# alebal123bal/BayesOpt_smart

Hardware: AMD Instinct MI355X
Metric: candidate-points/sec (GP predict + HVI) at N_train=512, N_cand=1M (higher is better)
Workload: dtype f64; 1 GPU; C3: 2D/2-obj toy_function, N_train=512, N_cand=1,048,576 per GPU ('ij' integer grid), HVI (Sigma-UCB), q=3; n_train=512, n_cand_per_gpu=1048576, n_cand_total=1048576, n_objectives=2, dim=2, topq=3, parallelism=candidate-shard x1, step_launch=hip_graph, candidate_offset=0

## Files before the change

### bayesopt_smart_amd/csrc/bo_gridconv.hip

```cpp

#include "bo_predict_impl.h"

namespace {

using namespace bo;

constexpr int kListWaves = 4;
constexpr int kListChunk = 512;
#ifndef BO_ACC_RB
#define BO_ACC_RB 8
#endif
constexpr int kAccRB = BO_ACC_RB;
constexpr int kAccRows = 64 * kAccRB;
constexpr int kAccUnroll = 4;
constexpr int kClassLists = kConvClasses * kConvShards;
static_assert(kClassLists % 64 == 0 && kClassLists <= 2 * 64 * kConvAccWaves &&
              (kConvShards & (kConvShards - 1)) == 0 && kConvShards <= 16 && kConvShards <= kConvCountStride,
              "conv_acc_kernel's scan and lookup of the class lists");
constexpr int kConvPF = 3;
constexpr size_t kConvLdsBytes = 160 * 1024;
constexpr double kPairDrop = 0x1p-100;
constexpr double kTabFlush = 0x1p-128;

struct ListLds {
  int order, rc, nm;
  size_t bytes;
  __host__ __device__ ListLds(int n, int C)
      : order(C + 1), rc(order + n), nm(rc + 2 * n), bytes((size_t)(nm + kListWaves * kListChunk) * sizeof(int)) {}
};
struct AccLds {
  int ints, part;
  size_t bytes;
  __host__ __device__ explicit AccLds(int R)
      : ints(4 * R), part(kClassLists + 1),
        bytes((size_t)ints * sizeof(double) + (size_t)(part + kConvAccWaves + 1) / 2 * 2 * sizeof(int)) {}
};
struct ContractLds {
  int HB, tabH, hband, cn;
  size_t bytes;
  __host__ __device__ ContractLds(int C, int Cpad, int LT, int NP)
      : HB(Cpad + LT / 2), tabH(2 * HB), hband(tabH + Cpad + C - 1), cn(hband + 1),
        bytes((size_t)cn * sizeof(double) + (size_t)NP * sizeof(int)) {}
};

__device__ __forceinline__ void conv_list_done(const ConvArgs& a, int tau, int kept, int lane, int dyn) {
  if (kept == 0) {
    for (int o = 0; o < a.n_obj; ++o) {
      double* row = a.T + ((size_t)o * a.LT + tau) * a.ldr;
      for (int i = lane; i < a.ldr; i += 64) row[i] = 0.0;
    }
  }
  if (lane == 0) {
    a.pkept[tau] = kept;
    if (dyn && kept > 0) {
      const int e = 31 - __clz(kept);
      const int cls = 2 * e + (e > 0 ? (kept >> (e - 1)) & 1 : 0);
      const int sh = tau & (kConvShards - 1);
      const int slot = atomicAdd(a.ccount + cls * kConvCountStride + sh, 1);
      a.clist[(size_t)(cls * kConvShards + sh) * (a.LT / kConvShards) + slot] = tau;
    }
  }
}

__global__ __launch_bounds__(64 * kListWaves) void conv_list_kernel(const ConvArgs a, int tau_blocks, int dyn) {
  if (__builtin_amdgcn_readfirstlane(*a.flag) != 0) return;
  const int tid = threadIdx.x;
  if ((int)blockIdx.x >= tau_blocks) {
    const long long total = (long long)a.NP * a.ldr;
    const long long stride = (long long)(gridDim.x - tau_blocks) * (64 * kListWaves);
    for (int o = 0; o < a.n_obj; ++o) {
      const double nhl = a.nhl[o], pv = a.pv[o];
      double* tm = a.Tm + (size_t)o * a.NP * a.ldr;
      for (long long t = (long long)(blockIdx.x - tau_blocks) * (64 * kListWaves) + tid; t < total; t += stride) {
        const int s = (int)(t / a.ldr), i = (int)(t - (long long)s * a.ldr);
        double v = 0.0;
        if (s < a.n && i < a.nrows) {
          const int n = a.order[s];
          const double d = (double)(a.row_lo + i - a.rc[2 * n]);
          v = pv * a.alpha[(size_t)o * a.n_pad + n] * exp(nhl * (d * d));
        }
        tm[t] = v;
      }
    }
    return;
  }
  extern __shared__ __attribute__((aligned(16))) int si[];
  const ListLds L(a.n, a.C);
  int* cstart = si;
  int* order = si + L.order;
  int* rc = si + L.rc;
  for (int t = tid; t <= a.C; t += 64 * kListWaves) cstart[t] = a.cstart[t];
  for (int t = tid; t < a.n; t += 64 * kListWaves) order[t] = a.order[t];
  for (int t = tid; t < 2 * a.n; t += 64 * kListWaves) rc[t] = a.rc[t];
  __syncthreads();
  const int lane = tid & 63, wave = tid >> 6;
// ... 185 lines not shown
    int incl = sum;
#pragma unroll
    for (int d = 1; d < 64; d <<= 1) {
      const int v = __shfl_up(incl, d, 64);
      if (lane >= d) incl += v;
    }
    if (lane == 63) part[tid >> 6] = incl;
    __syncthreads();
    int run = incl - sum;
    for (int w = 0; w < (tid >> 6); ++w) run += part[w];
#pragma unroll
    for (int u = 0; u < 2; ++u) {
      const int j = 2 * tid + u;
      if (j < kClassLists) cst[j] = run;
      run += c[u];
      if (j == kClassLists - 1) cst[kClassLists] = run;
    }
  }
  __syncthreads();
  const int n_items = (dyn ? cst[kClassLists] : a.LT) * nrb;
  const double* wo = pair_w + (size_t)o * a.n_pairs;
  const int g = blockIdx.x % ngrp;
  int* tk = ticket + (o * kConvTicketGroups + g) * kConvTicketStride;
  for (int k = (blockIdx.x / ngrp) * kConvAccWaves + (tid >> 6);;) {
    const int t = k * ngrp + g;
    if (t >= n_items) break;
    int nx = 0;
    if (dyn && lane == 0) nx = atomicAdd(tk, 1);
    const int oi = t / nrb, rb = t - oi * nrb;
    int tau = oi;
    if (dyn) {
      constexpr int per = kClassLists / 64;
      const unsigned long long b1 = __ballot(cst[per * lane + per] > oi);
      const int l1 = __builtin_ctzll(b1);
      const unsigned long long b2 = __ballot(cst[per * l1 + (lane < per ? lane : per - 1) + 1] > oi);
      const int j = per * l1 + __builtin_ctzll(b2);
      const int cls = kConvClasses - 1 - j / kConvShards;
      const int* list = clist + (size_t)(cls * kConvShards + j % kConvShards) * (a.LT / kConvShards);
      tau = __builtin_amdgcn_readfirstlane(list[oi - cst[j]]);
    }
    const int p0 = __builtin_amdgcn_readfirstlane(pstart[tau]);
    const int cnt = __builtin_amdgcn_readfirstlane(pkept[tau]);
    if (!dyn && cnt == 0) break;
    const int ib = rb * kAccRows;
    double* Trow = T + ((size_t)o * a.LT + tau) * a.ldr;
    if (ib + kAccRows <= a.nrows) conv_acc_item<true>(tabE, wo + p0, pair_sl + p0, cnt, ib, lane, a.nrows, a.ldr, Trow);
    else conv_acc_item<false>(tabE, wo + p0, pair_sl + p0, cnt, ib, lane, a.nrows, a.ldr, Trow);
    if (!dyn) break;
    k = __builtin_amdgcn_readfirstlane(nx);
  }
}

__device__ __forceinline__ void conv_load_a(const double* __restrict__ X, int ldr, int kb, int g, double (&v)[4]) {
  const double* p = X + (size_t)(16 * kb + 4 * g) * ldr;
#pragma unroll
  for (int s = 0; s < 4; ++s) v[s] = p[(size_t)s * ldr];
}

template <class BGen>
__device__ __forceinline__ void conv_gemm(const double* __restrict__ X, int ldr, int nkb, int g, d4 (&acc)[4],
                                          BGen&& bgen) {
  double ring[kConvPF][4];
#pragma unroll
  for (int p = 0; p < kConvPF; ++p) conv_load_a(X, ldr, p < nkb ? p : nkb - 1, g, ring[p]);
  for (int kb0 = 0; kb0 < nkb; kb0 += kConvPF) {
#pragma unroll
    for (int p = 0; p < kConvPF; ++p) {
      const int kb = kb0 + p;
      if (kb < nkb) {
        double av[4];
#pragma unroll
        for (int s = 0; s < 4; ++s) av[s] = ring[p][s];
        const int nx = kb + kConvPF;
        conv_load_a(X, ldr, nx < nkb ? nx : nkb - 1, g, ring[p]);
        double bv[4][4];
        bgen(kb, bv);
#pragma unroll
        for (int s = 0; s < 4; ++s)
#pragma unroll
          for (int nb = 0; nb < 4; ++nb) acc[nb] = mfma64(av[s], bv[s][nb], acc[nb]);
      }
    }
  }
}

__global__ __launch_bounds__(256, 2) void conv_contract_kernel(const ConvArgs a) {
  if (__builtin_amdgcn_readfirstlane(*a.flag) != 0) return;
  extern __shared__ __attribute__((aligned(16))) double sd[];
  const ContractLds L(a.C, a.Cpad, a.LT, a.NP);
  double* tabB = sd;
  double* tabH = sd + L.tabH;
  int* hband = (int*)(sd + L.hband);
  int* cn = (int*)(sd + L.cn);
  const int tid = threadIdx.x, lane = tid & 63, wave = tid >> 6;
  const int g = lane >> 4, jl = lane & 15;
  const int cb_n = a.Cpad / 64;
  const long long n_wt = (long long)(a.ldr / 16) * cb_n;
  const long long gi_lo = a.cand_offset, gi_hi = a.cand_offset + a.n_cand;
  for (int t = tid; t < a.NP; t += 256) cn[t] = t < a.n ? a.rc[2 * a.order[t] + 1] : 0;

  double lv = -__builtin_inf();
  long long li = -1;
  double tab_nhl = __builtin_nan("");
  for (long long base = (long long)blockIdx.x * 4; base < n_wt; base += (long long)gridDim.x * 4) {
    const long long wt = base + wave;
    const bool active = wt < n_wt;
    const long long wtc = active ? wt : n_wt - 1;
    const int i0 = (int)(wtc / cb_n) * 16, j0 = (int)(wtc % cb_n) * 64;
    double acq[4][4];
    for (int o = 0; o < a.n_obj; ++o) {
      const double nhl = a.nhl[o];
      if (!(nhl == tab_nhl)) {
        __syncthreads();
        int mq = 0;
        for (int t = tid; t < 2 * L.HB; t += 256) {
          const int par = t >= L.HB ? 1 : 0, h = t - par * L.HB;
          const int mi = 2 * h + par - (a.LT - 1);
          const double m = (double)mi;
          const double v = exp(0.5 * nhl * (m * m));
          const bool flush = v < kTabFlush;
          tabB[t] = flush ? 0.0 : v;
          if (!flush) mq = max(mq, abs(mi));
        }
        int mm = 0;
        for (int t = tid; t < a.Cpad + a.C - 1; t += 256) {
          const int mi = t - (a.C - 1);
          const double m = (double)mi;
          const double v = exp(nhl * (m * m));
          const bool flush = v < kTabFlush;
          tabH[t] = flush ? 0.0 : v;
          if (!flush) mm = max(mm, abs(mi));
        }
        if (tid < 2) hband[tid] = 0;
        __syncthreads();
#pragma unroll
        for (int d = 32; d > 0; d >>= 1) {
          mq = max(mq, __shfl_xor(mq, d, 64));
          mm = max(mm, __shfl_xor(mm, d, 64));
        }
        if (lane == 0) {
          atomicMax(hband, mq);
          atomicMax(hband + 1, mm);
        }
        __syncthreads();
        tab_nhl = nhl;
      }
      int kq_lo = 0, kq_hi = a.LT / 16;
      if (!a.full) {
        const int hq = hband[0];
        const int t_lo = 2 * j0 - hq > 0 ? 2 * j0 - hq : 0;
        const int t_hi = 2 * (j0 + 63) + hq < a.LT - 1 ? 2 * (j0 + 63) + hq : a.LT - 1;
        kq_lo = __builtin_amdgcn_readfirstlane(t_lo >> 4);
        kq_hi = __builtin_amdgcn_readfirstlane((t_hi >> 4) + 1);
      }
      d4 aq[4], am[4];
#pragma unroll
      for (int nb = 0; nb < 4; ++nb) {
        aq[nb] = (d4){0.0, 0.0, 0.0, 0.0};
        am[nb] = (d4){0.0, 0.0, 0.0, 0.0};
      }
      const double* Tq = a.T + ((size_t)o * a.LT + 16 * kq_lo) * a.ldr + i0 + jl;
      int km_lo = 0, km_hi = a.NP / 16;
      if (!a.full) {
        const int hm = hband[1];
        const int c_lo = j0 - hm > 0 ? j0 - hm : 0, c_hi = j0 + 64 + hm < a.C ? j0 + 64 + hm : a.C;
        km_lo = __builtin_amdgcn_readfirstlane(a.cstart[c_lo] >> 4);
        km_hi = __builtin_amdgcn_readfirstlane((a.cstart[c_hi] + 15) >> 4);
      }
      const double* Tm = a.Tm + ((size_t)o * a.NP + 16 * km_lo) * a.ldr + i0 + jl;
      const double* pe0 = tabB + (a.LT / 2 - 1 - 8 * kq_lo - 2 * g) + j0 + jl;
      conv_gemm(Tq, a.ldr, kq_hi - kq_lo, g, aq, [&](int kb, double (&bv)[4][4]) {
        const double* pe = pe0 - 8 * kb;
        const double* po = pe + L.HB;
#pragma unroll
        for (int nb = 0; nb < 4; ++nb) {
          bv[0][nb] = po[16 * nb];
          bv[1][nb] = pe[16 * nb];
          bv[2][nb] = po[16 * nb - 1];
          bv[3][nb] = pe[16 * nb - 1];
        }
      });
      const int* cn0 = cn + 16 * km_lo + 4 * g;
      if (km_hi > km_lo) conv_gemm(Tm, a.ldr, km_hi - km_lo, g, am, [&](int kb, double (&bv)[4][4]) {
        const int* c4 = cn0 + 16 * kb;
        const double* ph = tabH + j0 + jl + (a.C - 1);
#pragma unroll
        for (int s = 0; s < 4; ++s) {
          const double* p = ph - c4[s];
#pragma unroll
          for (int nb = 0; nb < 4; ++nb) bv[s][nb] = p[16 * nb];
        }
      });
      mfma_fence<false>(aq[0], aq[1]);
      mfma_fence<false>(aq[2], aq[3]);
      mfma_fence<false>(am[0], am[1]);
      mfma_fence<false>(am[2], am[3]);
      const double pv = a.pv[o], pm = a.pm[o];
#pragma unroll
      for (int nb = 0; nb < 4; ++nb) {
#pragma unroll
        for (int r = 0; r < 4; ++r) {
          const double mu = pm + am[nb][r];
          const double var = fmax(pv - aq[nb][r], a.min_var);
          const double smu = (mu - pm) * a.inv_rsq_pv[o];
          const double svar = var * a.inv_pv[o];
          const double u = smu + a.beta[o] * sqrt(fabs(svar));
          acq[nb][r] = (o == 0) ? u : acq[nb][r] + u;
          const int row = a.row_lo + i0 + g + 4 * r, c = j0 + 16 * nb + jl;
          const long long gi = (long long)row * a.C + c;
          if (active && i0 + g + 4 * r < a.nrows && c < a.C && gi >= gi_lo && gi < gi_hi) {
            const long long off = (long long)o * a.ld_out + (gi - gi_lo);
            if (a.mu) bo_out_store(a.mu + off, mu);
            if (a.var) bo_out_store(a.var + off, var);
            if (a.std_mu) bo_out_store(a.std_mu + off, smu);
            if (a.std_var) bo_out_store(a.std_var + off, svar);
            if (a.ucb) bo_out_store(a.ucb + off, u);
          }
        }
      }
    }
    long long gis[4][4];
#pragma unroll
    for (int nb = 0; nb < 4; ++nb) {
#pragma unroll
      for (int r = 0; r < 4; ++r) {
        const int row = a.row_lo + i0 + g + 4 * r, c = j0 + 16 * nb + jl;
        const long long gi = (long long)row * a.C + c;
        const bool ok = active && i0 + g + 4 * r < a.nrows && c < a.C && gi >= gi_lo && gi < gi_hi;
        gis[nb][r] = ok ? gi : -1;
        if (ok && a.acq) bo_out_store(a.acq + (gi - gi_lo), acq[nb][r]);
      }
    }
    if (a.topq > 0) {
      const int q = a.topq;
      const unsigned long long kq = bo_readlane_u(bo_order_key(lv, li), q - 1);
      const long long iq = bo_readlane_i(li, q - 1);
      bool beats = false;
#pragma unroll
      for (int nb = 0; nb < 4; ++nb)
#pragma unroll
        for (int r = 0; r < 4; ++r)
          beats = beats || bo_key_before(bo_order_key(acq[nb][r], gis[nb][r]), gis[nb][r], kq, iq);
      if (__ballot(beats) != 0ull) {
        unsigned int taken = 0;
        double nv = -__builtin_inf();
        long long ni = -1;
        int filled = 0;
        while (filled < q) {
          unsigned long long bk = 0ull;
          long long bi = -1;
          int bs = -1;
#pragma unroll
          for (int nb = 0; nb < 4; ++nb) {
#pragma unroll
            for (int r = 0; r < 4; ++r) {
              const int s = 4 * nb + r;
              const unsigned long long k = ((taken >> s) & 1u) ? 0ull : bo_order_key(acq[nb][r], gis[nb][r]);
              if (bo_key_before(k, gis[nb][r], bk, bi)) { bk = k; bi = gis[nb][r]; bs = s; }
            }
          }
          {
            const unsigned long long k = (lane < q && !((taken >> 16) & 1u)) ? bo_order_key(lv, li) : 0ull;
            if (bo_key_before(k, li, bk, bi)) { bk = k; bi = li; bs = 16; }
          }
          unsigned long long wk = bk;
          long long wi = bi;
#pragma unroll
          for (int m = 32; m > 0; m >>= 1) {
            const unsigned long long ok = __shfl_xor(wk, m, 64);
            const long long oi = __shfl_xor(wi, m, 64);
            if (bo_key_before(ok, oi, wk, wi)) { wk = ok; wi = oi; }
          }
          if (wk == 0ull) break;
          const bool win = bk == wk && bi == wi;
          bool excluded = false;
          if (win) {
            taken |= 1u << bs;
            if (bs != 16) {
              const long long row = wi / a.C, c = wi - row * a.C;
              double co[BO_MAX_DIM] = {(double)(a.lo0 + row), (double)(a.lo1 + c), 0.0, 0.0, 0.0, 0.0, 0.0, 0.0};
              excluded = bo_hash_contains(a.hkeys, a.hidx, a.hmask, a.excl_pts, 2, co, 2);
            }
          }
          if (__ballot(excluded) != 0ull) continue;
          if (lane == filled) { nv = bo_key_value(wk); ni = wi; }
          ++filled;
        }
        lv = nv;
        li = ni;
      }
    }
  }
  if (a.topq > 0) {
    if (lane < a.topq) {
      TopEntry* dst = a.partial + ((size_t)blockIdx.x * 4 + wave) * a.topq;
      dst[lane].v = lv;
      dst[lane].i = li;
    }
    if (blockIdx.x == 0) {
      const long long e0 = (long long)gridDim.x * 4 * a.topq, e1 = (long long)a.n_lists * a.topq;
      for (long long e = e0 + tid; e < e1; e += 256) {
        a.partial[e].v = -__builtin_inf();
        a.partial[e].i = -1;
      }
    }
  }
}

}

namespace bo {

bool conv_lds_admits(int n, int R, int C, int Cpad, int LT, int NP) {
  const size_t bound = ((size_t)4 * R + 2048) * sizeof(double) + ((size_t)(C + 1) + 3 * (size_t)n + 2048) * sizeof(int);
  assert(ConvSetupLds(n, C, 256).bytes <= bound && ListLds(n, C).bytes <= bound && AccLds(R).bytes <= bound);
  return bound <= kConvLdsBytes && ContractLds(C, Cpad, LT, NP).bytes <= kConvLdsBytes;
}

template <class K>
static hipError_t conv_lds_attr(K k, size_t lds) {
  if (lds <= 64 * 1024) return hipSuccess;
  return hipFuncSetAttribute((const void*)k, hipFuncAttributeMaxDynamicSharedMemorySize, (int)lds);
}

ConvSched conv_acc_schedule(int R, int LT, int ldr, int n_obj, int cus) {
  ConvSched sc;
  sc.nrb = (ldr + kAccRows - 1) / kAccRows;
  const long long items = (long long)LT * sc.nrb;
  const size_t tab = (size_t)4 * R * sizeof(double);
  const int per_cu = (int)(kConvLdsBytes / tab < 4 ? kConvLdsBytes / tab : 4);
  long long wgs = (long long)(cus > 0 ? cus : 256) * per_cu / n_obj;
  if (wgs > (items + kConvAccWaves - 1) / kConvAccWaves) wgs = (items + kConvAccWaves - 1) / kConvAccWaves;
  if (wgs < 1) wgs = 1;
  sc.wgs = (int)wgs;
  sc.ngrp = (int)(wgs < kConvTicketGroups ? wgs : kConvTicketGroups);
  sc.dyn = (items <= wgs * kConvAccWaves && wgs % sc.ngrp == 0) ? 0 : 1;
  return sc;
}

hipError_t launch_gridconv(const ConvArgs& ca, int grid, const ConvSched& sc, hipStream_t st) {
  const size_t l1 = ListLds(ca.n, ca.C).bytes, la = AccLds(ca.R).bytes;
  const size_t l2 = ContractLds(ca.C, ca.Cpad, ca.LT, ca.NP).bytes;
  if (l1 > kConvLdsBytes || la > kConvLdsBytes) return hipErrorInvalidValue;
  hipError_t e;
  if ((e = conv_lds_attr(conv_list_kernel, l1)) != hipSuccess) return e;
  if ((e = conv_lds_attr(conv_acc_kernel, la)) != hipSuccess) return e;
  if ((e = conv_lds_attr(conv_contract_kernel, l2)) != hipSuccess) return e;
  const int tau_blocks = (ca.LT + kListWaves - 1) / kListWaves;
  const long long tm_elems = (long long)ca.NP * ca.ldr;
  const int tm_blocks = (int)((tm_elems + 1023) / 1024 < 512 ? (tm_elems + 1023) / 1024 : 512);
  hipLaunchKernelGGL(conv_list_kernel, dim3(tau_blocks + tm_blocks), dim3(64 * kListWaves), l1, st, ca, tau_blocks,
                     sc.dyn);
  if ((e = hipGetLastError()) != hipSuccess) return e;
  hipLaunchKernelGGL(conv_acc_kernel, dim3((unsigned)sc.wgs, ca.n_obj), dim3(64 * kConvAccWaves), la, st, ca,
                     (const double*)ca.pair_w, (const int*)ca.pair_sl, (const int*)ca.pstart, (const int*)ca.pkept,
                     (const int*)ca.ccount, (const int*)ca.clist, ca.ticket, ca.T, sc.nrb, sc.ngrp, sc.dyn);
  if ((e = hipGetLastError()) != hipSuccess) return e;
  hipLaunchKernelGGL(conv_contract_kernel, dim3(grid), dim3(256), l2, st, ca);
  return hipGetLastError();
}

}
```

### bayesopt_smart_amd/csrc/bo_predict.hip

```cpp

#include "bo_predict_impl.h"

#include <vector>

namespace {

__device__ __forceinline__ double kstar_at(const FusedArgs& a, int o, int f, long long j, bool valid) {
  return (valid && f < a.n_train) ? a.kstar[((long long)o * a.ks_rows + f) * a.n_cand + j] : 0.0;
}

template <int NS, bool SELECT>
__device__ __forceinline__ void contract_epair(__amdgpu_buffer_rsrc_t wr, int voff, int base,
                                               int& pos, int ep, const double (&B)[NS],
                                               d2 (&wa)[kPF], d2 (&wb)[kPF], d4& acc0, d4& acc1,
                                               double (&sel0)[4], double (&sel1)[4]) {
  constexpr int NCH = NS / 8;
#pragma unroll
  for (int c = 0; c < NCH; ++c) {
#pragma unroll
    for (int pp = 0; pp < 4; ++pp) {
      const int p = 4 * c + pp;
      const d2 ca = wa[pp];
      const d2 cb = wb[pp];
      const int so = base + ((pos + kPF) << 11);
// ... 353 lines not shown
  if (b < p.alpha_blocks) {
    const long long row_id = (long long)b * 4 + wave;
    if (row_id >= (long long)p.n_obj * p.n_pad) return;
    const int o = (int)(row_id / p.n_pad), f = (int)(row_id % p.n_pad);
    double s = 0.0;
    if (f < p.n) {
      const double* wr = p.kinv + (long long)o * p.ld_k * p.ld_k + (long long)f * p.ld_k;
      const double pm = p.pm[o];
      for (int e = lane; e < p.n; e += 64) s = __builtin_fma(wr[e], p.y[(long long)e * p.ld_y + o] - pm, s);
    }
#pragma unroll
    for (int m = 32; m > 0; m >>= 1) s += __shfl_xor(s, m, 64);
    if (lane == 0) p.alpha[row_id] = s;
    return;
  }
  b -= p.alpha_blocks;
  const long long t0 = (long long)b * 256 + tid, stride = (long long)p.pack_blocks * 256;
  if (p.pack_mode == 0) pack_cm_range(t0, stride, (d2*)p.wpack, p.kinv, p.ld_k, p.upper, p.n, p.n_pad, p.n_obj);
  else if (p.pack_mode == 1) pack_range(t0, stride, (d2*)p.wpack, p.kinv, p.ld_k, p.n, p.n_pad, p.ns, p.n_obj);
  else pack32_range(t0, stride, (f4*)p.wpack, p.kinv, p.ld_k, p.n, p.n_pad, p.n_obj);
}

__global__ void selftest_mfma32_kernel(const float* a, const float* b, float* d) {
  const int l = threadIdx.x;
  const float av = a[(l & 15) * 4 + (l >> 4)];
  const float bv = b[(l >> 4) * 16 + (l & 15)];
  f4 acc = {0.0f, 0.0f, 0.0f, 0.0f};
  acc = mfma32(av, bv, acc);
#pragma unroll
  for (int r = 0; r < 4; ++r) d[(4 * (l >> 4) + r) * 16 + (l & 15)] = acc[r];
}

inline int pad_rows(long long n) { return (int)((n + 31) / 32 * 32); }
inline int pad_dim(int d) { return d <= 2 ? 2 : (d <= 4 ? 4 : (d <= 6 ? 6 : 8)); }
inline size_t align256(size_t x) { return (x + 255) & ~(size_t)255; }
constexpr size_t kLdsBytes = 160 * 1024;
constexpr size_t kLdsDoubles = kLdsBytes / sizeof(double);

int num_cus() {
  static int cus = 0;
  if (cus == 0) {
    int dev = 0;
    if (hipGetDevice(&dev) != hipSuccess) return 256;
    hipDeviceProp_t p;
    if (hipGetDeviceProperties(&p, dev) != hipSuccess) return 256;
    cus = p.multiProcessorCount;
  }
  return cus;
}

constexpr double kConvMargin = 1.15;
constexpr int kConvMaxN = 4096;

void plan_gridconv(const bo_predict_desc* d, Plan* pl, bool kmem) {
  if (kmem || !pl->cm || d->cand_kind != BO_CAND_GRID || d->dim != 2 || d->n_cand <= 0) return;
  if (d->mode & (BO_PREDICT_DENSE | BO_PREDICT_NO_SEPARABLE | BO_PREDICT_FP32 | BO_PREDICT_NO_GRID_CONV)) return;
  const char* env = getenv("BO_GRID_CONV");
  if (env && env[0] == '0' && env[1] == 0) return;
  const long long R = d->grid_shape[0], C = d->grid_shape[1], n = d->n_train;
  if (R < 1 || C < 1 || R > (1 << 15) || C > (1 << 15) || n > kConvMaxN) return;
  if (d->cand_offset < 0 || d->cand_offset + d->n_cand > R * C) return;
  bo::ConvPlan cp = {};
  cp.row_lo = (int)(d->cand_offset / C);
  cp.nrows = (int)((d->cand_offset + d->n_cand - 1) / C) - cp.row_lo + 1;
  cp.ldr = (cp.nrows + 15) / 16 * 16;
  cp.Cpad = (int)((C + 63) / 64 * 64);
  cp.LT = (int)((2 * C - 1 + 15) / 16 * 16);
  cp.NP = (int)((n + 15) / 16 * 16);
  if (!bo::conv_lds_admits((int)n, (int)R, (int)C, cp.Cpad, cp.LT, cp.NP)) return;
  const long long wave_tiles = (long long)(cp.ldr / 16) * (cp.Cpad / 64);
  if (!(d->mode & (BO_PREDICT_GRID_CONV | BO_PREDICT_GRID_CONV_FULL))) {
    const double nch = pl->n_pad / 32;
    const double F = (double)d->n_obj * 1024.0 * nch * (nch + 1);
    const double old_rounds = (double)(((d->n_cand + 63) / 64 + 255) / 256);
    const double old_us = 25.0 + old_rounds * 64.0 * (F / 273.0e3 + 0.038);
    const double pairs_per_tau = 0.5 * (double)n * (double)(n + 1) / (double)(2 * C - 1);
    const double pair_us = 2.2 * pairs_per_tau * (double)((cp.ldr + 1023) / 1024) *
                           (double)((d->n_obj * (2 * C - 1) + 4095) / 4096);
    const double tile_rounds = (double)((wave_tiles + 1023) / 1024);
    const double contract_us = tile_rounds * 2048.0 * (double)(cp.LT + cp.NP) * (double)d->n_obj / 48.8e3;
    const double conv_us = 60.0 + pair_us + contract_us;
    if (!(kConvMargin * conv_us < old_us)) return;
  }
  cp.planned = true;
  const long long wgs = (wave_tiles + 3) / 4;
  cp.grid = (int)(wgs < pl->grid ? wgs : pl->grid);
  cp.ws = bo::conv_layout(n, d->n_obj, C, cp.LT, cp.NP, cp.ldr, align256(pl->total));
  pl->total = cp.ws.end;
  pl->conv = cp;
}

int make_plan(const bo_predict_desc* d, Plan* pl, bool query_device, bool kmem = false) {
  if (!d || d->n_obj < 1 || d->n_obj > BO_MAX_OBJ || d->dim < 1 || d->dim > BO_MAX_DIM)
    return BO_ERR_ARG;
  if (d->n_train < 1 || d->n_cand < 0 || d->topq < 0 || d->topq > BO_MAX_TOPQ) return BO_ERR_ARG;
  if (d->cand_kind < 0 || d->cand_kind > BO_CAND_SOBOL) return BO_ERR_ARG;
  if (d->mode & ~(BO_PREDICT_DENSE | BO_PREDICT_NO_SEPARABLE | BO_PREDICT_FP32 | BO_PREDICT_F32_FLOOR |
                  BO_PREDICT_NO_GRID_CONV | BO_PREDICT_GRID_CONV | BO_PREDICT_GRID_CONV_FULL))
    return BO_ERR_ARG;
  if (d->excl_points && d->n_excl < 0) return BO_ERR_ARG;
  const long long n = d->n_train;
  if (n > (1 << 14)) return BO_ERR_UNSUPPORTED;
  memset(pl, 0, sizeof(*pl));
  pl->dim_pad = pad_dim(d->dim);
  pl->n_excl = (int)(d->excl_points ? d->n_excl : n);
  pl->n_panels = 1;
  if ((d->mode & BO_PREDICT_FP32) && !kmem) {
    const int n_pad = (int)((n + 63) / 64 * 64);
    const size_t lds = ((size_t)n_pad * pl->dim_pad + (size_t)d->n_obj * n_pad) * sizeof(float);
    if (lds <= kLdsBytes) {
      pl->fp32 = true;
      pl->n_pad = n_pad;
      pl->ns = 16;
      pl->lds = lds;
    }
  }
  if (!pl->fp32 && !kmem) {
    const int n_pad = pad_rows(n);
    const size_t base = (size_t)n_pad * pl->dim_pad + (size_t)d->n_obj * n_pad;
    pl->cm = true;
    pl->n_pad = n_pad;
    pl->ns = n_pad / 4;
    const size_t plain = base + bo::kExpTab;
    size_t lds = plain;
    if (d->cand_kind == BO_CAND_GRID && !(d->mode & BO_PREDICT_NO_SEPARABLE)) {
      const long long S = d->grid_shape[d->dim - 1];
      const size_t tbl = (size_t)d->n_obj * (2 * S - 1);
      const size_t rw_c = (size_t)n_pad * (d->n_obj + 1) + (size_t)(S + 63) / 64;
      const size_t lds_c = base + tbl + (size_t)kWaves * rw_c;
      const size_t lds_1 = base + tbl + (size_t)kWaves * n_pad * 2;
      if (S % 16 == 0 && S <= 32768 && d->cand_offset % 16 == 0 && lds_1 <= kLdsDoubles) {
        pl->sep = true;
        pl->rw_cache = lds_c <= kLdsDoubles;
        pl->rw_stride = (int)(pl->rw_cache ? rw_c : (size_t)n_pad * 2);
        pl->off_tbl = (int)base;
        pl->off_rw = (int)(base + tbl);
        lds = pl->rw_cache ? lds_c : lds_1;
        if (lds < plain) lds = plain;
      }
    }
    pl->off_exp = (int)base;
    if (lds > kLdsDoubles) {
      pl->sep = false;
      pl->grows = true;
      pl->off_exp = 0;
      lds = bo::kExpTab;
    }
    pl->lds = lds * sizeof(double);
#ifndef BO_ABL_NOSMALL
    pl->small = !pl->grows && n_pad <= 4 * 32 && pl->lds <= kLdsBytes / 2 - 1024;
#endif
  }
  if (kmem) {
    int n_pad = pad_rows(n);
    int ns;
    bool multi = false;
    if (n_pad <= 32) ns = 8;
    else if (n_pad <= 64) ns = 16;
    else if (n_pad <= 128) ns = 32;
    else if (n_pad <= 256) ns = 64;
    else { ns = bo::kPanelSteps; multi = true; }
    n_pad = multi ? (int)((n + 511) / 512 * 512) : ns * 4;
    pl->n_pad = n_pad;
    pl->ns = ns;
    pl->multi = multi;
    pl->n_panels = multi ? n_pad / 512 : 1;
    pl->lds = (size_t)d->n_obj * n_pad * sizeof(double);
    if (pl->lds > 160 * 1024) return BO_ERR_UNSUPPORTED;
  }
  const int n_pad = pl->n_pad;
  const size_t w_bytes = (size_t)d->n_obj * n_pad * n_pad * sizeof(double);
  if (w_bytes >= (1ull << 31)) return BO_ERR_UNSUPPORTED;
  pl->waves = kWaves;
  const long long n_tiles = (d->n_cand + kTile - 1) / kTile;
  pl->n_tiles = n_tiles;
  const int cus = query_device ? num_cus() : 256;
#ifdef BO_SMALL_ONE_SLOT
  const int slots = cus;
#else
  const int slots = pl->small ? 2 * cus : cus;
#endif
  pl->grid = (int)(n_tiles < slots ? (n_tiles > 0 ? n_tiles : 1) : slots);
  pl->off_alpha = align256(w_bytes);
  pl->off_xpad = pl->off_alpha + align256((size_t)d->n_obj * n_pad * sizeof(double));
  pl->off_xc = pl->off_xpad + align256((size_t)n_pad * pl->dim_pad * sizeof(double));
  pl->off_excl = pl->off_xc + align256((size_t)n_pad * pl->dim_pad * sizeof(double));
  pl->off_hash = pl->off_excl + align256((size_t)(pl->n_excl + 1) * pl->dim_pad * sizeof(double));
  pl->hash_slots = bo_hash_slots(pl->n_excl);
  pl->off_partial = pl->off_hash + align256((size_t)pl->hash_slots * 12);
  pl->off_status = pl->off_partial +
                   align256((size_t)1024 * kWaves * (d->topq > 0 ? d->topq : 1) * sizeof(TopEntry));
  pl->total = pl->off_status + 256 + 256;
  plan_gridconv(d, pl, kmem);
  return BO_OK;
}

template <int NS, bool MULTI>
hipError_t launch_kmem_k(const FusedArgs& fa, int grid, size_t lds, hipStream_t st) {
  auto k = kmem_predict_kernel<NS, MULTI>;
  if (lds > 64 * 1024) {
    hipError_t e = hipFuncSetAttribute((const void*)k, hipFuncAttributeMaxDynamicSharedMemorySize,
                                       (int)lds);
    if (e != hipSuccess) return e;
  }
  hipLaunchKernelGGL(k, dim3(grid), dim3(256), lds, st, fa);
  return hipGetLastError();
}

hipError_t launch_kmem(const Plan& pl, const FusedArgs& fa, hipStream_t s) {
  if (pl.multi) return launch_kmem_k<bo::kPanelSteps, true>(fa, pl.grid, pl.lds, s);
  switch (pl.ns) {
    case 8: return launch_kmem_k<8, false>(fa, pl.grid, pl.lds, s);
    case 16: return launch_kmem_k<16, false>(fa, pl.grid, pl.lds, s);
    case 32: return launch_kmem_k<32, false>(fa, pl.grid, pl.lds, s);
    default: return launch_kmem_k<64, false>(fa, pl.grid, pl.lds, s);
  }
}

struct KernelTimer {
  bool on = false;
  int used = 0;
  std::vector<hipEvent_t> ev;
} g_timer;

void timer_mark(hipStream_t s) {
  if (!g_timer.on || g_timer.used >= (int)g_timer.ev.size()) return;
  (void)hipEventRecord(g_timer.ev[g_timer.used++], s);
}

}

extern "C" {

size_t bo_predict_workspace_size(const bo_predict_desc* d) {
  Plan pl;
  if (make_plan(d, &pl, false) != BO_OK) return 0;
  return pl.total;
}

static int validate_call(const bo_predict_desc* d, const Plan& pl, bool kmem, const void* workspace, size_t ws_bytes) {
  if (!workspace || ws_bytes < pl.total) return BO_ERR_WORKSPACE;
  if ((!kmem && !d->x_train) || !d->y_train || !d->kinv || d->ld_k < d->n_train ||
      d->ld_y < d->n_obj)
    return BO_ERR_ARG;
  if (d->cand_kind != BO_CAND_GRID && d->n_cand > 0 && !d->cand) return BO_ERR_ARG;
  if (d->topq > 0 && (!d->top_val || !d->top_idx)) return BO_ERR_ARG;
// ... 174 lines not shown
  pa.DIM = pl.dim_pad;
  pa.sep_flag = (int*)fa.sep_flag;
  pa.sep_lo = fa.sep_lo;
  pa.sep_S = fa.sep_S;
  pa.excl = (double*)(ws + pl.off_excl);
  pa.excl_in = d->excl_points;
  pa.n_excl = (kmem || !d->excl_points) ? 0 : pl.n_excl;
  pa.hkeys = (unsigned long long*)fa.hkeys;
  pa.hidx = (int*)fa.hidx;
  pa.hslots = pl.hash_slots;
  pa.n_hash = (kmem || d->topq == 0) ? 0 : pl.n_excl;
  pa.hash_lds = pa.n_hash > 0 && pl.hash_slots <= 2048 ? 1 : 0;
  return pa.hash_lds ? (size_t)pl.hash_slots * 12 : 0;
}

static int predict_impl(const bo_predict_desc* d, const double* kstar, long long ks_rows,
                        void* workspace, size_t ws_bytes, void* stream) {
  const bool kmem = kstar != nullptr;
  Plan pl;
  int st = make_plan(d, &pl, true, kmem);
  if (st != BO_OK) return st;
  if ((st = validate_call(d, pl, kmem, workspace, ws_bytes)) != BO_OK) return st;
  hipStream_t s = (hipStream_t)stream;
  char* ws = (char*)(((uintptr_t)workspace + 255) & ~(uintptr_t)255);

  FusedArgs fa;
  if ((st = fill_fused_args(d, pl, ws, kstar, ks_rows, fa)) != BO_OK) return st;
  PrepArgs pa;
  size_t prep_lds = fill_prep_args(d, pl, ws, kmem, fa, pa);
  const bo::ConvArgs& ca = pa.conv;
  if (pl.conv.planned) {
    fill_conv_args(d, pl, ws, fa, pa.conv);
    pa.sched = bo::conv_acc_schedule(ca.R, ca.LT, ca.ldr, ca.n_obj, num_cus());
    const size_t setup_lds = bo::ConvSetupLds(ca.n, ca.C, 256).bytes;
    if (setup_lds > prep_lds) prep_lds = setup_lds;
  }
  if (prep_lds > 64 * 1024)
    BO_CHECK_HIP(hipFuncSetAttribute((const void*)predict_prep_kernel, hipFuncAttributeMaxDynamicSharedMemorySize,
                                     (int)prep_lds));
  hipLaunchKernelGGL(predict_prep_kernel,
                     dim3((unsigned)(2 + (pl.conv.planned ? 1 : 0) + pa.alpha_blocks + pa.pack_blocks)), dim3(256),
                     prep_lds, s, pa);
  BO_CHECK_HIP(hipGetLastError());
  if (d->n_cand == 0) {
    if (d->topq > 0) {
      BO_CHECK_HIP(hipMemsetAsync(d->top_idx, 0xff, sizeof(int64_t) * d->topq, s));
    }
    return BO_OK;
  }
  hipError_t e;
  const bool timed = g_timer.on && g_timer.used + 2 <= (int)g_timer.ev.size();
  if (timed) timer_mark(s);
  if (pl.conv.planned) {
    if (bo::launch_gridconv(ca, pl.conv.grid, pa.sched, s) != hipSuccess) return BO_ERR_HIP;
  }
  if (kmem) e = launch_kmem(pl, fa, s);
  else if (pl.fp32) switch (pl.dim_pad) {
    case 2: e = bo::launch_c32_d2(pl, fa, s); break;
    case 4: e = bo::launch_c32_d4(pl, fa, s); break;
    case 6: e = bo::launch_c32_d6(pl, fa, s); break;
    default: e = bo::launch_c32_d8(pl, fa, s); break;
  }
  else switch (pl.dim_pad) {
    case 2: e = bo::launch_cm_d2(pl, fa, s); break;
    case 4: e = bo::launch_cm_d4(pl, fa, s); break;
    case 6: e = bo::launch_cm_d6(pl, fa, s); break;
    default: e = bo::launch_cm_d8(pl, fa, s); break;
  }
  if (e != hipSuccess) return BO_ERR_HIP;
  if (timed) timer_mark(s);
  if (d->topq > 0) {
    const long long nl = (long long)pl.grid * pl.waves;
    if (!bo_launch_rounds_merge(fa.partial, nl, d->topq, d->top_val, d->top_idx, s)) {
      hipLaunchKernelGGL(bo_topq_merge_kernel, dim3(1), dim3(256), 0, s, fa.partial, nl, d->topq, d->top_val,
                         (long long*)d->top_idx);
      BO_CHECK_HIP(hipGetLastError());
    }
  }
  return BO_OK;
}

int bo_predict_acquire(const bo_predict_desc* d, void* workspace, size_t ws_bytes, void* stream) {
  return predict_impl(d, nullptr, 0, workspace, ws_bytes, stream);
}

static void fill_mv_desc(bo_predict_desc* d, int32_t n_obj, int64_t n_cand, int64_t n) {
  memset(d, 0, sizeof(*d));
  d->n_obj = n_obj;
  d->dim = 1;
  d->n_train = n;
  d->cand_kind = BO_CAND_GRID;
  d->n_cand = n_cand;
  d->grid_shape[0] = n_cand > 0 ? n_cand : 1;
  d->n_excl = 0;
  d->mode = BO_PREDICT_DENSE;
}

size_t bo_update_mean_variance_workspace_size(int32_t n_obj, int64_t current_eval) {
  bo_predict_desc d;
  fill_mv_desc(&d, n_obj, 0, current_eval);
  d.excl_points = (const double*)1;
  Plan pl;
  if (make_plan(&d, &pl, false, true) != BO_OK) return 0;
  return pl.total;
}

int bo_update_mean_variance(double* mu, double* var, const double* k_star, int64_t ld_rows,
// ... 67 lines not shown
```

### bayesopt_smart_amd/csrc/bo_predict_impl.h

```cpp
#pragma once

#include "bo_common.h"

#include <assert.h>
#include <math.h>
#include <stdlib.h>
#include <string.h>

#include <type_traits>

namespace bo {

constexpr int kWaves = 4;
constexpr int kTile = 16 * kWaves;
constexpr int kPanelSteps = 128;
constexpr int kPF = 4;
constexpr int kCMaxEp = 16;
constexpr int kC32MaxEp = 16;
constexpr int kExpTab = 256;

struct FusedArgs {
  int n_obj, dim, n_train, n_pad;
  int n_panels;
  int n_excl;
// ... 156 lines not shown
    unsigned long long m = __ballot(valid);
    for (int b = 0; b < bits; ++b) {
      const bool bit = (c >> b) & 1;
      const unsigned long long bal = __ballot(valid && bit);
      m &= bit ? bal : ~bal;
    }
    const unsigned long long below = m & ((1ull << lane) - 1ull);
    const int base = valid ? cnt[c] : 0;
    __builtin_amdgcn_fence(__ATOMIC_RELEASE, "wavefront");
    __builtin_amdgcn_wave_barrier();
    __builtin_amdgcn_fence(__ATOMIC_ACQUIRE, "wavefront");
    if (valid) {
      a.order[base + __popcll(below)] = n;
      if (below == 0ull) cnt[c] = base + __popcll(m);
    }
    __builtin_amdgcn_fence(__ATOMIC_RELEASE, "wavefront");
    __builtin_amdgcn_wave_barrier();
    __builtin_amdgcn_fence(__ATOMIC_ACQUIRE, "wavefront");
  }
}

struct ConvLayout {
  size_t cstart, order, rc, pstart, pkept, clist, ticket, ccount, Tm, T, pair_sl, pair_w, end;
};

inline ConvLayout conv_layout(long long n, int n_obj, long long C, long long LT, long long NP, long long ldr,
                              size_t base) {
  size_t at = base;
  auto take = [&at](long long count, size_t elem, size_t align) {
    const size_t off = (at + align - 1) / align * align;
    at = off + (size_t)count * elem;
    return off;
  };
  const long long pairs = n * (n + 1) / 2;
  ConvLayout L;
  L.cstart = take(C + 1, sizeof(int), 256);
  L.order = take(n, sizeof(int), sizeof(int));
  L.rc = take(2 * n, sizeof(int), sizeof(int));
  L.pstart = take(LT, sizeof(int), sizeof(int));
  L.pkept = take(LT, sizeof(int), sizeof(int));
  L.clist = take(kConvClasses * LT, sizeof(int), sizeof(int));
  L.ticket = take(BO_MAX_OBJ * kConvTicketGroups * kConvTicketStride, sizeof(int), 128);
  L.ccount = take(kConvClasses * kConvCountStride, sizeof(int), 128);
  L.Tm = take(n_obj * NP * ldr, sizeof(double), 256);
  L.T = take(n_obj * LT * ldr, sizeof(double), 256);
  L.pair_sl = take(pairs, sizeof(int), 256);
  L.pair_w = take(n_obj * pairs, sizeof(double), 256);
  L.end = take(0, 1, 256) + (L.ticket % 256 == 0 ? 256 : 0);
  return L;
}

bool conv_lds_admits(int n, int R, int C, int Cpad, int LT, int NP);
ConvSched conv_acc_schedule(int R, int LT, int ldr, int n_obj, int cus);
hipError_t launch_gridconv(const ConvArgs& ca, int grid, const ConvSched& sc, hipStream_t st);

struct ConvPlan {
  bool planned;
  int grid;
  int row_lo, nrows, ldr, LT, NP, Cpad;
  ConvLayout ws;
};

struct Plan {
  int n_pad, ns, n_panels, dim_pad, n_excl;
  bool multi;
  size_t off_alpha, off_xpad, off_xc, off_excl, off_hash, off_partial, off_status, total;
  unsigned int hash_slots;
  bool cm;
  bool sep;
  bool grows;
  int off_tbl, off_rw;
  bool rw_cache;
  int rw_stride;
  bool fp32;
  bool small;
  int off_exp;
  int grid, waves;
  long long n_tiles;
  size_t lds;
  ConvPlan conv;
};

hipError_t launch_cm_d2(const Plan& pl, const FusedArgs& fa, hipStream_t st);
hipError_t launch_cm_d4(const Plan& pl, const FusedArgs& fa, hipStream_t st);
hipError_t launch_cm_d6(const Plan& pl, const FusedArgs& fa, hipStream_t st);
hipError_t launch_cm_d8(const Plan& pl, const FusedArgs& fa, hipStream_t st);
hipError_t launch_c32_d2(const Plan& pl, const FusedArgs& fa, hipStream_t st);
hipError_t launch_c32_d4(const Plan& pl, const FusedArgs& fa, hipStream_t st);
hipError_t launch_c32_d6(const Plan& pl, const FusedArgs& fa, hipStream_t st);
hipError_t launch_c32_d8(const Plan& pl, const FusedArgs& fa, hipStream_t st);
hipError_t launch_cms_d2(const Plan& pl, const FusedArgs& fa, hipStream_t st);
hipError_t launch_cms_d4(const Plan& pl, const FusedArgs& fa, hipStream_t st);
hipError_t launch_cms_d6(const Plan& pl, const FusedArgs& fa, hipStream_t st);
hipError_t launch_cms_d8(const Plan& pl, const FusedArgs& fa, hipStream_t st);

}

namespace {

using bo::FusedArgs;
using bo::Plan;
using bo::kWaves;
using bo::kTile;
using bo::kPF;
using bo::kCMaxEp;
using bo::kC32MaxEp;
using bo::kExpTab;

template <int DIM>
__device__ __forceinline__ void load_candidate(const FusedArgs& a, long long j, bool valid,
                                               double (&c)[DIM]) {
#pragma unroll
  for (int k = 0; k < DIM; ++k) c[k] = 0.0;
  if (!valid) return;
// ... 970 lines not shown
```

Baseline: 5.212 billion candidate-points/sec.

## Adapt grid-conv contract tile width and waves per block, merge top-q per block

Templates the contract kernel on the tile width (16/32/64 columns) and lets the planner pick it, along with 4 or 8 waves per block, based on tile count versus CU count. The grid is capped at one block per CU. Per-wave top-q lists are merged in LDS so each block writes a single list, which shrinks the partials the final reduction reads. It also adds several ablation macros that are off by default. The aim is better load balance and occupancy on the contract stage, at the cost of less B-operand reuse with narrower tiles and an extra intra-block merge.

```diff
diff --git a/bayesopt_smart_amd/csrc/bo_gridconv.hip b/bayesopt_smart_amd/csrc/bo_gridconv.hip
--- a/bayesopt_smart_amd/csrc/bo_gridconv.hip
+++ b/bayesopt_smart_amd/csrc/bo_gridconv.hip
@@ -17,7 +17,11 @@
 static_assert(kClassLists % 64 == 0 && kClassLists <= 2 * 64 * kConvAccWaves &&
               (kConvShards & (kConvShards - 1)) == 0 && kConvShards <= 16 && kConvShards <= kConvCountStride,
               "conv_acc_kernel's scan and lookup of the class lists");
-constexpr int kConvPF = 3;
+#ifndef BO_CONV_PF
+#define BO_CONV_PF 3
+#endif
+constexpr int kConvPF = BO_CONV_PF;
+constexpr int kContractWaves = 8;
 constexpr size_t kConvLdsBytes = 160 * 1024;
 constexpr double kPairDrop = 0x1p-100;
 constexpr double kTabFlush = 0x1p-128;
@@ -38,9 +42,11 @@
 struct ContractLds {
   int HB, tabH, hband, cn;
   size_t bytes;
-  __host__ __device__ ContractLds(int C, int Cpad, int LT, int NP)
+  __host__ __device__ ContractLds(int C, int Cpad, int LT, int NP, int lists = 0)
       : HB(Cpad + LT / 2), tabH(2 * HB), hband(tabH + Cpad + C - 1), cn(hband + 1),
-        bytes((size_t)cn * sizeof(double) + (size_t)NP * sizeof(int)) {}
+        bytes((size_t)cn * sizeof(double) + (size_t)NP * sizeof(int)) {
+    if (bytes < (size_t)lists * sizeof(TopEntry)) bytes = (size_t)lists * sizeof(TopEntry);
+  }
 };
 
 __device__ __forceinline__ void conv_list_done(const ConvArgs& a, int tau, int kept, int lane, int dyn) {
@@ -332,13 +338,18 @@
 }
 
 __device__ __forceinline__ void conv_load_a(const double* __restrict__ X, int ldr, int kb, int g, double (&v)[4]) {
+#ifdef BO_ABL_CT_ACONST
+#pragma unroll
+  for (int s = 0; s < 4; ++s) v[s] = X[0];
+#else
   const double* p = X + (size_t)(16 * kb + 4 * g) * ldr;
 #pragma unroll
   for (int s = 0; s < 4; ++s) v[s] = p[(size_t)s * ldr];
-}
-
-template <class BGen>
-__device__ __forceinline__ void conv_gemm(const double* __restrict__ X, int ldr, int nkb, int g, d4 (&acc)[4],
+#endif
+}
+
+template <int NB, class BGen>
+__device__ __forceinline__ void conv_gemm(const double* __restrict__ X, int ldr, int nkb, int g, d4 (&acc)[NB],
                                           BGen&& bgen) {
   double ring[kConvPF][4];
 #pragma unroll
@@ -353,18 +364,19 @@
         for (int s = 0; s < 4; ++s) av[s] = ring[p][s];
         const int nx = kb + kConvPF;
         conv_load_a(X, ldr, nx < nkb ? nx : nkb - 1, g, ring[p]);
-        double bv[4][4];
+        double bv[4][NB];
         bgen(kb, bv);
 #pragma unroll
         for (int s = 0; s < 4; ++s)
 #pragma unroll
-          for (int nb = 0; nb < 4; ++nb) acc[nb] = mfma64(av[s], bv[s][nb], acc[nb]);
-      }
-    }
-  }
-}
-
-__global__ __launch_bounds__(256, 2) void conv_contract_kernel(const ConvArgs a) {
+          for (int nb = 0; nb < NB; ++nb) acc[nb] = mfma64(av[s], bv[s][nb], acc[nb]);
+      }
+    }
+  }
+}
+
+template <int NB>
+__global__ __launch_bounds__(64 * kContractWaves) void conv_contract_kernel(const ConvArgs a) {
   if (__builtin_amdgcn_readfirstlane(*a.flag) != 0) return;
   extern __shared__ __attribute__((aligned(16))) double sd[];
   const ContractLds L(a.C, a.Cpad, a.LT, a.NP);
@@ -372,28 +384,37 @@
   double* tabH = sd + L.tabH;
   int* hband = (int*)(sd + L.hband);
   int* cn = (int*)(sd + L.cn);
+  constexpr int TW = 16 * NB;
   const int tid = threadIdx.x, lane = tid & 63, wave = tid >> 6;
+  const int nt = blockDim.x, W = nt >> 6;
   const int g = lane >> 4, jl = lane & 15;
-  const int cb_n = a.Cpad / 64;
+  const int cb_n = a.Cpad / TW;
   const long long n_wt = (long long)(a.ldr / 16) * cb_n;
   const long long gi_lo = a.cand_offset, gi_hi = a.cand_offset + a.n_cand;
-  for (int t = tid; t < a.NP; t += 256) cn[t] = t < a.n ? a.rc[2 * a.order[t] + 1] : 0;
+#ifndef BO_ABL_CT_NOOUT
+  const bool outs = true;
+#else
+  const bool outs = a.ld_out < 0;
+#endif
+  for (int t = tid; t < a.NP; t += nt) cn[t] = t < a.n ? a.rc[2 * a.order[t] + 1] : 0;
 
   double lv = -__builtin_inf();
   long long li = -1;
   double tab_nhl = __builtin_nan("");
-  for (long long base = (long long)blockIdx.x * 4; base < n_wt; base += (long long)gridDim.x * 4) {
+  for (long long base = (long long)blockIdx.x * W; base < n_wt; base += (long long)gridDim.x * W) {
     const long long wt = base + wave;
     const bool active = wt < n_wt;
     const long long wtc = active ? wt : n_wt - 1;
-    const int i0 = (int)(wtc / cb_n) * 16, j0 = (int)(wtc % cb_n) * 64;
-    double acq[4][4];
+    const int i0 = (int)(wtc / cb_n) * 16, j0 = (int)(wtc % cb_n) * TW;
+    double acq[NB][4];
     for (int o = 0; o < a.n_obj; ++o) {
       const double nhl = a.nhl[o];
       if (!(nhl == tab_nhl)) {
         __syncthreads();
         int mq = 0;
-        for (int t = tid; t < 2 * L.HB; t += 256) {
+        int mm = 0;
+#ifndef BO_ABL_CT_NOTAB
+        for (int t = tid; t < 2 * L.HB; t += nt) {
           const int par = t >= L.HB ? 1 : 0, h = t - par * L.HB;
           const int mi = 2 * h + par - (a.LT - 1);
           const double m = (double)mi;
@@ -402,8 +423,7 @@
           tabB[t] = flush ? 0.0 : v;
           if (!flush) mq = max(mq, abs(mi));
         }
-        int mm = 0;
-        for (int t = tid; t < a.Cpad + a.C - 1; t += 256) {
+        for (int t = tid; t < a.Cpad + a.C - 1; t += nt) {
           const int mi = t - (a.C - 1);
           const double m = (double)mi;
           const double v = exp(nhl * (m * m));
@@ -411,6 +431,10 @@
           tabH[t] = flush ? 0.0 : v;
           if (!flush) mm = max(mm, abs(mi));
         }
+#else
+        mm = min((int)sqrt(128.0 * 0.6931471805599453 / -nhl), a.C - 1);
+        mq = min((int)sqrt(256.0 * 0.6931471805599453 / -nhl), a.LT - 1);
+#endif
         if (tid < 2) hband[tid] = 0;
         __syncthreads();
 #pragma unroll
@@ -428,14 +452,14 @@
       int kq_lo = 0, kq_hi = a.LT / 16;
       if (!a.full) {
         const int hq = hband[0];
-        const int t_lo = 2 * j0 - hq > 0 ? 2 * j0 - hq : 0;
-        const int t_hi = 2 * (j0 + 63) + hq < a.LT - 1 ? 2 * (j0 + 63) + hq : a.LT - 1;
+        const int t_hi = 2 * (j0 + TW - 1) + hq < a.LT - 1 ? 2 * (j0 + TW - 1) + hq : a.LT - 1;
+        const int t_lo = 2 * j0 - hq > 0 ? (2 * j0 - hq < t_hi ? 2 * j0 - hq : t_hi) : 0;
         kq_lo = __builtin_amdgcn_readfirstlane(t_lo >> 4);
         kq_hi = __builtin_amdgcn_readfirstlane((t_hi >> 4) + 1);
       }
-      d4 aq[4], am[4];
-#pragma unroll
-      for (int nb = 0; nb < 4; ++nb) {
+      d4 aq[NB], am[NB];
+#pragma unroll
+      for (int nb = 0; nb < NB; ++nb) {
         aq[nb] = (d4){0.0, 0.0, 0.0, 0.0};
         am[nb] = (d4){0.0, 0.0, 0.0, 0.0};
       }
@@ -443,41 +467,64 @@
       int km_lo = 0, km_hi = a.NP / 16;
       if (!a.full) {
         const int hm = hband[1];
-        const int c_lo = j0 - hm > 0 ? j0 - hm : 0, c_hi = j0 + 64 + hm < a.C ? j0 + 64 + hm : a.C;
+        const int c_hi = j0 + TW + hm < a.C ? j0 + TW + hm : a.C;
+        const int c_lo = j0 - hm > 0 ? (j0 - hm < a.C ? j0 - hm : a.C) : 0;
         km_lo = __builtin_amdgcn_readfirstlane(a.cstart[c_lo] >> 4);
         km_hi = __builtin_amdgcn_readfirstlane((a.cstart[c_hi] + 15) >> 4);
       }
       const double* Tm = a.Tm + ((size_t)o * a.NP + 16 * km_lo) * a.ldr + i0 + jl;
       const double* pe0 = tabB + (a.LT / 2 - 1 - 8 * kq_lo - 2 * g) + j0 + jl;
-      conv_gemm(Tq, a.ldr, kq_hi - kq_lo, g, aq, [&](int kb, double (&bv)[4][4]) {
+#ifdef BO_ABL_CT_BCONST
+      const double bconst = pe0[0];
+#endif
+      conv_gemm<NB>(Tq, a.ldr, kq_hi - kq_lo, g, aq, [&](int kb, double (&bv)[4][NB]) {
+#ifdef BO_ABL_CT_BCONST
+#pragma unroll
+        for (int s = 0; s < 4; ++s)
+#pragma unroll
+          for (int nb = 0; nb < NB; ++nb) bv[s][nb] = bconst;
+#else
         const double* pe = pe0 - 8 * kb;
         const double* po = pe + L.HB;
 #pragma unroll
-        for (int nb = 0; nb < 4; ++nb) {
+        for (int nb = 0; nb < NB; ++nb) {
           bv[0][nb] = po[16 * nb];
           bv[1][nb] = pe[16 * nb];
           bv[2][nb] = po[16 * nb - 1];
           bv[3][nb] = pe[16 * nb - 1];
         }
+#endif
       });
       const int* cn0 = cn + 16 * km_lo + 4 * g;
-      if (km_hi > km_lo) conv_gemm(Tm, a.ldr, km_hi - km_lo, g, am, [&](int kb, double (&bv)[4][4]) {
+      if (km_hi > km_lo) conv_gemm<NB>(Tm, a.ldr, km_hi - km_lo, g, am, [&](int kb, double (&bv)[4][NB]) {
+#ifdef BO_ABL_CT_BCONST
+#pragma unroll
+        for (int s = 0; s < 4; ++s)
+#pragma unroll
+          for (int nb = 0; nb < NB; ++nb) bv[s][nb] = bconst;
+#else
         const int* c4 = cn0 + 16 * kb;
         const double* ph = tabH + j0 + jl + (a.C - 1);
 #pragma unroll
         for (int s = 0; s < 4; ++s) {
           const double* p = ph - c4[s];
 #pragma unroll
-          for (int nb = 0; nb < 4; ++nb) bv[s][nb] = p[16 * nb];
-        }
+          for (int nb = 0; nb < NB; ++nb) bv[s][nb] = p[16 * nb];
+        }
+#endif
       });
-      mfma_fence<false>(aq[0], aq[1]);
-      mfma_fence<false>(aq[2], aq[3]);
-      mfma_fence<false>(am[0], am[1]);
-      mfma_fence<false>(am[2], am[3]);
+      if constexpr (NB == 1) {
+        mfma_fence<false>(aq[0], am[0]);
+      } else {
+#pragma unroll
+        for (int nb = 0; nb < NB; nb += 2) {
+          mfma_fence<false>(aq[nb], aq[nb + 1]);
+          mfma_fence<false>(am[nb], am[nb + 1]);
+        }
+      }
       const double pv = a.pv[o], pm = a.pm[o];
 #pragma unroll
-      for (int nb = 0; nb < 4; ++nb) {
+      for (int nb = 0; nb < NB; ++nb) {
 #pragma unroll
         for (int r = 0; r < 4; ++r) {
           const double mu = pm + am[nb][r];
@@ -488,7 +535,7 @@
           acq[nb][r] = (o == 0) ? u : acq[nb][r] + u;
           const int row = a.row_lo + i0 + g + 4 * r, c = j0 + 16 * nb + jl;
           const long long gi = (long long)row * a.C + c;
-          if (active && i0 + g + 4 * r < a.nrows && c < a.C && gi >= gi_lo && gi < gi_hi) {
+          if (outs && active && i0 + g + 4 * r < a.nrows && c < a.C && gi >= gi_lo && gi < gi_hi) {
             const long long off = (long long)o * a.ld_out + (gi - gi_lo);
             if (a.mu) bo_out_store(a.mu + off, mu);
             if (a.var) bo_out_store(a.var + off, var);
@@ -499,25 +546,30 @@
         }
       }
     }
-    long long gis[4][4];
-#pragma unroll
-    for (int nb = 0; nb < 4; ++nb) {
+    long long gis[NB][4];
+#pragma unroll
+    for (int nb = 0; nb < NB; ++nb) {
 #pragma unroll
       for (int r = 0; r < 4; ++r) {
         const int row = a.row_lo + i0 + g + 4 * r, c = j0 + 16 * nb + jl;
         const long long gi = (long long)row * a.C + c;
         const bool ok = active && i0 + g + 4 * r < a.nrows && c < a.C && gi >= gi_lo && gi < gi_hi;
         gis[nb][r] = ok ? gi : -1;
-        if (ok && a.acq) bo_out_store(a.acq + (gi - gi_lo), acq[nb][r]);
-      }
-    }
-    if (a.topq > 0) {
+        if (outs && ok && a.acq) bo_out_store(a.acq + (gi - gi_lo), acq[nb][r]);
+      }
+    }
+#ifndef BO_ABL_CT_NOSEL
+    const bool select = a.topq > 0;
+#else
+    const bool select = a.topq > 0 && a.n_lists < 0;
+#endif
+    if (select) {
       const int q = a.topq;
       const unsigned long long kq = bo_readlane_u(bo_order_key(lv, li), q - 1);
       const long long iq = bo_readlane_i(li, q - 1);
       bool beats = false;
 #pragma unroll
-      for (int nb = 0; nb < 4; ++nb)
+      for (int nb = 0; nb < NB; ++nb)
 #pragma unroll
         for (int r = 0; r < 4; ++r)
           beats = beats || bo_key_before(bo_order_key(acq[nb][r], gis[nb][r]), gis[nb][r], kq, iq);
@@ -531,7 +583,7 @@
           long long bi = -1;
           int bs = -1;
 #pragma unroll
-          for (int nb = 0; nb < 4; ++nb) {
+          for (int nb = 0; nb < NB; ++nb) {
 #pragma unroll
             for (int r = 0; r < 4; ++r) {
               const int s = 4 * nb + r;
@@ -572,14 +624,46 @@
     }
   }
   if (a.topq > 0) {
-    if (lane < a.topq) {
-      TopEntry* dst = a.partial + ((size_t)blockIdx.x * 4 + wave) * a.topq;
-      dst[lane].v = lv;
-      dst[lane].i = li;
+    const int q = a.topq;
+    TopEntry* ml = (TopEntry*)sd;
+    __syncthreads();
+    if (lane < q) {
+      ml[wave * q + lane].v = lv;
+      ml[wave * q + lane].i = li;
+    }
+    __syncthreads();
+    if (wave == 0) {
+      int head = 0;
+      double nv = -__builtin_inf();
+      long long ni = -1;
+      for (int r = 0; r < q; ++r) {
+        const bool has = lane < W && head < q;
+        const double hv = has ? ml[lane * q + head].v : -__builtin_inf();
+        const long long hi = has ? ml[lane * q + head].i : -1;
+        const unsigned long long bk = bo_order_key(hv, hi);
+        unsigned long long wk = bk;
+        long long wi = hi;
+#pragma unroll
+        for (int m = 32; m > 0; m >>= 1) {
+          const unsigned long long ok = __shfl_xor(wk, m, 64);
+          const long long oi = __shfl_xor(wi, m, 64);
+          if (bo_key_before(ok, oi, wk, wi)) { wk = ok; wi = oi; }
+        }
+        if (wk == 0ull) break;
+        const bool win = bk == wk && hi == wi;
+        if (win) ++head;
+        const double wv = __shfl(hv, __builtin_ctzll(__ballot(win)), 64);
+        if (lane == r) { nv = wv; ni = wi; }
+      }
+      if (lane < q) {
+        TopEntry* dst = a.partial + (size_t)blockIdx.x * q;
+        dst[lane].v = nv;
+        dst[lane].i = ni;
+      }
     }
     if (blockIdx.x == 0) {
-      const long long e0 = (long long)gridDim.x * 4 * a.topq, e1 = (long long)a.n_lists * a.topq;
-      for (long long e = e0 + tid; e < e1; e += 256) {
+      const long long e0 = (long long)gridDim.x * q, e1 = (long long)a.n_lists * q;
+      for (long long e = e0 + tid; e < e1; e += nt) {
         a.partial[e].v = -__builtin_inf();
         a.partial[e].i = -1;
       }
@@ -618,14 +702,16 @@
   return sc;
 }
 
-hipError_t launch_gridconv(const ConvArgs& ca, int grid, const ConvSched& sc, hipStream_t st) {
+hipError_t launch_gridconv(const ConvArgs& ca, const ConvPlan& cp, const ConvSched& sc, hipStream_t st) {
   const size_t l1 = ListLds(ca.n, ca.C).bytes, la = AccLds(ca.R).bytes;
-  const size_t l2 = ContractLds(ca.C, ca.Cpad, ca.LT, ca.NP).bytes;
+  const size_t l2 = ContractLds(ca.C, ca.Cpad, ca.LT, ca.NP, cp.waves * ca.topq).bytes;
   if (l1 > kConvLdsBytes || la > kConvLdsBytes) return hipErrorInvalidValue;
+  if (cp.waves < 1 || cp.waves > kContractWaves || cp.grid > ca.n_lists) return hipErrorInvalidValue;
+  auto* contract = cp.nb == 4 ? conv_contract_kernel<4> : cp.nb == 2 ? conv_contract_kernel<2> : conv_contract_kernel<1>;
   hipError_t e;
   if ((e = conv_lds_attr(conv_list_kernel, l1)) != hipSuccess) return e;
   if ((e = conv_lds_attr(conv_acc_kernel, la)) != hipSuccess) return e;
-  if ((e = conv_lds_attr(conv_contract_kernel, l2)) != hipSuccess) return e;
+  if ((e = conv_lds_attr(contract, l2)) != hipSuccess) return e;
   const int tau_blocks = (ca.LT + kListWaves - 1) / kListWaves;
   const long long tm_elems = (long long)ca.NP * ca.ldr;
   const int tm_blocks = (int)((tm_elems + 1023) / 1024 < 512 ? (tm_elems + 1023) / 1024 : 512);
@@ -636,7 +722,7 @@
                      (const double*)ca.pair_w, (const int*)ca.pair_sl, (const int*)ca.pstart, (const int*)ca.pkept,
                      (const int*)ca.ccount, (const int*)ca.clist, ca.ticket, ca.T, sc.nrb, sc.ngrp, sc.dyn);
   if ((e = hipGetLastError()) != hipSuccess) return e;
-  hipLaunchKernelGGL(conv_contract_kernel, dim3(grid), dim3(256), l2, st, ca);
+  hipLaunchKernelGGL(contract, dim3(cp.grid), dim3(64 * cp.waves), l2, st, ca);
   return hipGetLastError();
 }
 
diff --git a/bayesopt_smart_amd/csrc/bo_predict.hip b/bayesopt_smart_amd/csrc/bo_predict.hip
--- a/bayesopt_smart_amd/csrc/bo_predict.hip
+++ b/bayesopt_smart_amd/csrc/bo_predict.hip
@@ -429,7 +429,7 @@
 constexpr double kConvMargin = 1.15;
 constexpr int kConvMaxN = 4096;
 
-void plan_gridconv(const bo_predict_desc* d, Plan* pl, bool kmem) {
+void plan_gridconv(const bo_predict_desc* d, Plan* pl, bool kmem, int cus) {
   if (kmem || !pl->cm || d->cand_kind != BO_CAND_GRID || d->dim != 2 || d->n_cand <= 0) return;
   if (d->mode & (BO_PREDICT_DENSE | BO_PREDICT_NO_SEPARABLE | BO_PREDICT_FP32 | BO_PREDICT_NO_GRID_CONV)) return;
   const char* env = getenv("BO_GRID_CONV");
@@ -460,8 +460,22 @@
     if (!(kConvMargin * conv_us < old_us)) return;
   }
   cp.planned = true;
-  const long long wgs = (wave_tiles + 3) / 4;
-  cp.grid = (int)(wgs < pl->grid ? wgs : pl->grid);
+  const long long tiles64 = wave_tiles;
+  cp.nb = tiles64 >= 8LL * cus ? 4 : 2 * tiles64 >= 8LL * cus ? 2 : 1;
+  const char* tile = getenv("BO_CONV_TILE");
+  if (tile && (tile[0] == '1' || tile[0] == '2' || tile[0] == '4') && tile[1] == 0) cp.nb = tile[0] - '0';
+  const long long tiles = tiles64 * (4 / cp.nb);
+  cp.waves = tiles >= 8LL * cus ? 8 : 4;
+  long long wgs = (tiles + cp.waves - 1) / cp.waves;
+#ifdef BO_ABL_CT_W4
+  cp.waves = 4;
+  wgs = (tiles + 3) / 4;
+  if (wgs > 2LL * cus) wgs = 2LL * cus;
+#else
+  if (wgs > cus) wgs = cus;
+#endif
+  if (wgs > (long long)pl->grid * pl->waves) wgs = (long long)pl->grid * pl->waves;
+  cp.grid = (int)wgs;
   cp.ws = bo::conv_layout(n, d->n_obj, C, cp.LT, cp.NP, cp.ldr, align256(pl->total));
   pl->total = cp.ws.end;
   pl->conv = cp;
@@ -568,7 +582,7 @@
   pl->off_status = pl->off_partial +
                    align256((size_t)1024 * kWaves * (d->topq > 0 ? d->topq : 1) * sizeof(TopEntry));
   pl->total = pl->off_status + 256 + 256;
-  plan_gridconv(d, pl, kmem);
+  plan_gridconv(d, pl, kmem, cus);
   return BO_OK;
 }
 
@@ -849,7 +863,7 @@
   const bool timed = g_timer.on && g_timer.used + 2 <= (int)g_timer.ev.size();
   if (timed) timer_mark(s);
   if (pl.conv.planned) {
-    if (bo::launch_gridconv(ca, pl.conv.grid, pa.sched, s) != hipSuccess) return BO_ERR_HIP;
+    if (bo::launch_gridconv(ca, pl.conv, pa.sched, s) != hipSuccess) return BO_ERR_HIP;
   }
   if (kmem) e = launch_kmem(pl, fa, s);
   else if (pl.fp32) switch (pl.dim_pad) {
diff --git a/bayesopt_smart_amd/csrc/bo_predict_impl.h b/bayesopt_smart_amd/csrc/bo_predict_impl.h
--- a/bayesopt_smart_amd/csrc/bo_predict_impl.h
+++ b/bayesopt_smart_amd/csrc/bo_predict_impl.h
@@ -232,14 +232,17 @@
 
 bool conv_lds_admits(int n, int R, int C, int Cpad, int LT, int NP);
 ConvSched conv_acc_schedule(int R, int LT, int ldr, int n_obj, int cus);
-hipError_t launch_gridconv(const ConvArgs& ca, int grid, const ConvSched& sc, hipStream_t st);
 
 struct ConvPlan {
   bool planned;
+  int nb;
+  int waves;
   int grid;
   int row_lo, nrows, ldr, LT, NP, Cpad;
   ConvLayout ws;
 };
+
+hipError_t launch_gridconv(const ConvArgs& ca, const ConvPlan& cp, const ConvSched& sc, hipStream_t st);
 
 struct Plan {
   int n_pad, ns, n_panels, dim_pad, n_excl;
```

New measurement: 5.439 billion candidate-points/sec (median of 6 runs). +4.4%, better.
